# caidj0/Raytracer-2025

Hardware: NVIDIA B200
Metric: paths_per_sec (higher is better)
Workload: dtype f64

## Files before the change

### raytracer-2025_b200/csrc/api.cu

```cuda
#include <cuda_runtime.h>

#include <algorithm>
#include <cstdio>
#include <cstdlib>
#include <cstring>
#include <memory>
#include <mutex>
#include <new>
#include <string>
#include <thread>
#include <vector>

#include "compile.h"
#include "kernels.h"
#include "rt2025.h"

using namespace rt;

namespace {

thread_local std::string g_err;

int set_err(int code, const std::string& msg) {
    g_err = msg;
// ... 255 lines not shown
            if (!cs.nodes4.empty() && cs.nodes.size() * sizeof(Node) <= 2 * budget && stacks + cs.nodes4.size() * sizeof(Node4) > budget &&
                !getenv("RT2025_WIDE_BVH")) {
                RawVec<Node4>().swap(cs.nodes4);
                cs.world_root4 = INVALID_REF;
            }
        }
        s = new rt_scene();
        s->device = device;
        s->sm_count = sms;
        SceneView& v = s->view;
        keep_pool_memory(device);
        {
            cudaStream_t st = cudaStreamPerThread;
            Arena a;
            a.reserve(cs.nodes4), a.reserve(cs.nodes), a.reserve(cs.geom), a.reserve(cs.meta), a.reserve(cs.xforms), a.reserve(cs.materials), a.reserve(cs.textures);
            a.reserve(cs.images), a.reserve(cs.texels), a.reserve(cs.perlins), a.reserve(cs.media), a.reserve(cs.lights), a.reserve(cs.remaps);
            a.allocate(st);
            s->arena = a.base;
            v.nodes4 = a.put(cs.nodes4, st), v.world_root4 = cs.world_root4;
            v.nodes = a.put(cs.nodes, st), v.geom = a.put(cs.geom, st), v.meta = a.put(cs.meta, st), v.xforms = a.put(cs.xforms, st);
            v.materials = a.put(cs.materials, st), v.textures = a.put(cs.textures, st), v.images = a.put(cs.images, st);
            v.texels = a.put(cs.texels, st), v.perlins = a.put(cs.perlins, st), v.media = a.put(cs.media, st);
            v.lights = a.put(cs.lights, st), v.remaps = a.put(cs.remaps, st);
            CU(cudaStreamSynchronize(st));
        }
        v.world_root = cs.world_root;
        v.n_media = (uint32_t)cs.media.size();
        v.n_xforms = (uint32_t)cs.xforms.size();
        v.kinds = (cs.n_spheres && !cs.n_planars) ? 1u : ((cs.n_planars && !cs.n_spheres) ? 2u : 0u);
        v.n_lights = (uint32_t)cs.lights.size();
        v.n_prims = (uint32_t)cs.geom.size();
        s->ranks = cs.ranks;
        for (auto& m : cs.media) s->generic_media |= m.single_sphere == RT_NONE;
        v.media_xform = 0;
        for (auto& m : cs.media)
            if (m.xform != RT_NONE || (m.single_sphere != RT_NONE && cs.meta[m.single_sphere].xform != RT_NONE)) v.media_xform = 1;
        for (auto& m : cs.materials) s->class_mask |= 1u << m.shade_class;
        for (auto& t : cs.textures) s->black_texture.push_back(t.kind == RT_TEX_SOLID && t.color[0] == 0.0 && t.color[1] == 0.0 && t.color[2] == 0.0);
// ... 377 lines not shown
        CU(cudaEventRecord(ev[1], st));
        CU(cudaEventSynchronize(ev[1]));
        CU(cudaGetLastError());
        if (stats) {
            float ms = 0;
            CU(cudaEventElapsedTime(&ms, ev[0], ev[1]));
            const Counters zero{};
            const Counters& c = final_counters ? *final_counters : zero;
            stats->paths = nominal_paths;
            stats->segments = total_paths ? c.segments : 0;
            stats->node_visits = total_paths ? c.node_visits : 0;
            stats->prim_tests = total_paths ? c.prim_tests : 0;
            stats->errors = total_paths ? c.errors : 0;
            stats->iterations = total_paths ? c.iterations : 0;
            stats->reserved[0] = total_paths ? c.walk_segments : 0;
            stats->kernel_launches = launches;
            stats->ms_total = ms;
            stats->ms_raygen = ms_gen, stats->ms_extend = ms_ext, stats->ms_shade = ms_shd;
            stats->ms_other = ms_med;
        }
    } catch (const CudaFail& f) {
        rc = set_err(RT_ERR_CUDA, f.what);
    }
    for (auto& e : ev)
        if (e) cudaEventDestroy(e);
    return rc;
}

int rt_render(const rt_scene* s, const rt_camera* cam, const rt_render_opts* opts, void* accum, rt_stats* stats) {
    if (!s || !cam || !accum) return set_err(RT_ERR_INVALID, "null argument");
// ... 272 lines not shown
```

### raytracer-2025_b200/csrc/compile.cpp

```cpp
#include "compile.h"

#include <omp.h>

#include <memory>
#include <parallel/algorithm>

#include <chrono>
#include <cstdio>
#include <cstdlib>

#include <vector_functions.h>

#include <algorithm>
#include <cmath>
#include <cstring>
#include <limits>

namespace rt {

namespace {

struct V3 {
    double x, y, z;
};
// ... 968 lines not shown
            Medium& med = out.media[m];
            med.n_entry = MEDIUM_NO_ENTRIES;
            if (!(med.flags & MEDIUM_THICK) || getenv("RT2025_WALK_NO_ENTRIES")) continue;
            GroupBox b = group_boxes[group_of_medium[m]];
            for (int k = 0; k < 3; k++) {
                const float pad = 1e-4f * std::max(1.0f, std::max(std::fabs(b.lo[k]), std::fabs(b.hi[k])));
                b.lo[k] -= pad, b.hi[k] += pad;
            }
            uint32_t n = 0;
            const double* g = out.geom[med.single_sphere].d;
            const bool plain = med.xform == RT_NONE && out.meta[med.single_sphere].xform == RT_NONE && g[3] == 0.0 && g[4] == 0.0 && g[5] == 0.0;
            const double ball[4] = {g[0], g[1], g[2], std::fabs(g[6]) * (1.0 + 1e-4) + 1e-4};
            if (overlapping_leaves(b, plain ? ball : nullptr, out.world_root, med.entry, n)) med.n_entry = n;
            if (timer.on) fprintf(stderr, "[rt2025 compile] medium %zu is optically thick: %d entry leaves\n", m, (int)med.n_entry);
        }
        return RT_OK;
    }
};

}

int compile_scene(const rt_scene_desc& d, uint32_t flags, CompiledScene& out, std::string& err, WorldBuilder world_builder) {
    Compiler c{d, flags, out, err};
    c.world_builder = world_builder;
    return c.run();
}

}
```

### raytracer-2025_b200/csrc/compile.h

```cpp
#pragma once
#include <memory>
#include <string>
#include <type_traits>
#include <utility>
#include <vector>

#include <vector_types.h>

#include "rt2025.h"
#include "scene_types.h"

namespace rt {

template <class T, class A = std::allocator<T>>
struct default_init_allocator : A {
    using A::A;
    template <class U>
    struct rebind {
        using other = default_init_allocator<U, typename std::allocator_traits<A>::template rebind_alloc<U>>;
    };
    template <class U>
    void construct(U* p) noexcept(std::is_nothrow_default_constructible<U>::value) {
        ::new (static_cast<void*>(p)) U;
    }
// ... 10 lines not shown
    RawVec<Node4> nodes4;
    uint32_t world_root4 = INVALID_REF;
    uint32_t bvh4_depth = 0;
    RawVec<PrimGeom> geom;
    RawVec<PrimMeta> meta;
    std::vector<Xform> xforms;
    std::vector<Material> materials;
    std::vector<Texture> textures;
    std::vector<Image> images;
    std::vector<float4> texels;
    std::vector<Perlin> perlins;
    std::vector<Medium> media;
    std::vector<Light> lights;
    std::vector<Remap> remaps;
    std::vector<uint32_t> ranks;
    uint32_t world_root = INVALID_REF;
    uint32_t bvh_depth = 0;
    uint32_t media_bvh_depth = 0;
    uint32_t n_spheres = 0, n_planars = 0;
};

struct BuildBox;
using WorldBuilder = bool (*)(const RawVec<BuildBox>& boxes, uint32_t first_prim_base, RawVec<Node>& nodes,
                              RawVec<uint32_t>& order, uint32_t& depth_out, uint32_t& root_out);

int compile_scene(const rt_scene_desc& d, uint32_t flags, CompiledScene& out, std::string& err, WorldBuilder world_builder = nullptr);

uint32_t collapse_bvh4(const RawVec<Node>& nodes, uint32_t root, RawVec<Node4>& out, uint32_t& depth_out);

struct BuildBox {
// ... 9 lines not shown
```

### raytracer-2025_b200/csrc/kernels.cu

```cuda
#include <cuda_runtime.h>
#include <stdint.h>

#include <algorithm>

#include "kernels.h"
#include "shade.cuh"

namespace rt {

struct RayArrayIO {
    const SceneView& sv;
    const rt_ray* __restrict__ rays;
    rt_hit* __restrict__ out;
    double tmin, tmax;
    __device__ __forceinline__ double t_min() const { return tmin; }
    __device__ __forceinline__ bool load(uint32_t i, RayD& r, double& t1, uint32_t& prim0, uint32_t& rank0) const {
        const double* rp = reinterpret_cast<const double*>(rays + i);
        r.o = D3{rp[0], rp[1], rp[2]};
        r.d = D3{rp[3], rp[4], rp[5]};
        r.time = rp[6];
        t1 = tmax;
        prim0 = 0xFFFFFFFFu, rank0 = 0xFFFFFFFFu;
        return true;
    }
// ... 163 lines not shown
struct MediumDraws {
    Rand2 pair;
    uint32_t slot = 0xFFFFFFFFu;
    __device__ __forceinline__ double get(uint64_t seed, uint32_t pixel, uint32_t sample, uint32_t segment, uint32_t medium_index) {
        const uint32_t s = RT_MEDIUM_SLOT(medium_index);
        if (s != slot) {
            pair = philox_pair(seed, pixel, sample, segment, s);
            slot = s;
        }
        return (medium_index & 1u) ? pair.b : pair.a;
    }
};

constexpr uint32_t MEDIUM_INCUMBENT = 0x80000000u;

template <bool COUNT, bool XF>
__device__ __forceinline__ bool sample_sphere_medium(const SceneView& sv, const Medium& med, const RayD& r, double xi, double& tm, TraceCounters* cnt) {
    RayD lr = r;
    if (XF && med.xform != RT_NONE) lr = ray_to_local(sv, med.xform, r);
    RayD br = lr;
    if (XF) {
        const uint32_t bx = sv.meta[med.single_sphere].xform;
        if (bx != med.xform) br = bx == RT_NONE ? r : ray_to_local(sv, bx, r);
    }
    double t1, t2;
    if (COUNT) cnt->prims += 2;
    if (!sphere_entry_exit(sv.geom[med.single_sphere].d, br, t1, t2)) return false;
    if (t1 < 1e-8) t1 = 1e-8;
    if (t1 >= t2) return false;
    if (t1 < 0.0) t1 = 0.0;
    const double ray_length = length(lr.d);
    const double distance_inside_boundary = (t2 - t1) * ray_length;
    const float hf = (float)med.neg_inv_density * logf((float)xi);
    const float hf_err = 4e-7f * fabsf((float)med.neg_inv_density);
    if (hf > (float)distance_inside_boundary * 1.001f + hf_err) return false;
    const double hit_distance = med.neg_inv_density * log(xi);
    if (hit_distance > distance_inside_boundary) return false;
    tm = t1 + hit_distance / ray_length;
    return true;
}

template <bool COUNT, int MEDIA>
struct PathIO {
    const SceneView& sv;
    const RayRec* __restrict__ rays;
    HitRec* __restrict__ hits;
    uint8_t* __restrict__ cls;
    uint64_t seed;
    bool bin_by_class, drop_misses;
    TraceCounters* cnt;
    __device__ __forceinline__ double t_min() const { return 1e-8; }
    __device__ __forceinline__ bool load(uint32_t j, RayD& r, double& t1, uint32_t& prim0, uint32_t& rank0) const {
        uint64_t ids;
        load_ray(rays + j, r, ids);
// ... 70 lines not shown
template <bool COUNT, bool GENERIC, bool XF, int FILTER = 0>
__device__ __forceinline__ bool sample_media(const SceneView& sv, uint64_t seed, const RayD& r, uint32_t pixel, uint32_t sample, uint32_t segment, double& t,
                                             uint32_t& prim, uint32_t& kind, const float4* s_mem, uint32_t* stack, int stride, TraceCounters* cntp,
                                             uint32_t first, MediumDraws& draws) {
    uint32_t rank = kind == HIT_SURFACE ? sv.meta[prim].rank : (kind == HIT_MEDIUM ? sv.media[prim].rank : 0xFFFFFFFFu);
    bool changed = false;
        for (uint32_t k = 0; k < sv.n_media; k++) {
            uint32_t m = first + k;
            if (m >= sv.n_media) m -= sv.n_media;
            if (FILTER && ((sv.media[m].flags & MEDIUM_THICK) != 0u) != (FILTER == 1)) continue;
            const Medium& med = sv.media[m];
            const double xi = draws.get(seed, pixel, sample, segment, med.medium_index);
            double tm;
            RayD lr = r;
            if (XF && med.xform != RT_NONE) lr = ray_to_local(sv, med.xform, r);
            if (RT_MEDIA_EARLY_SCREEN && kind != HIT_MISS) {
                const float hf = (float)med.neg_inv_density * logf((float)xi);
                const float hf_err = 4e-7f * fabsf((float)med.neg_inv_density);
                const float len_f = sqrtf((float)lr.d.x * (float)lr.d.x + (float)lr.d.y * (float)lr.d.y + (float)lr.d.z * (float)lr.d.z);
                if (hf > (float)t * len_f * 1.001f + hf_err) continue;
            }
            if (med.single_sphere != RT_NONE) {
                if (!sample_sphere_medium<COUNT, XF>(sv, med, r, xi, tm, cntp)) continue;
            } else if (GENERIC) {
                double t1, t2;
                uint32_t bp;
                if (!closest_hit<COUNT, false>(sv, med.root, r, -INFINITY, INFINITY, s_mem, stack, stride, t1, bp, cntp)) continue;
                if (!closest_hit<COUNT, false>(sv, med.root, r, t1 + 0.0001, INFINITY, s_mem, stack, stride, t2, bp, cntp)) continue;
                if (t1 < 1e-8) t1 = 1e-8;
                if (t1 >= t2) continue;
                if (t1 < 0.0) t1 = 0.0;
                const double ray_length = length(lr.d);
                const double distance_inside_boundary = (t2 - t1) * ray_length;
                const double hit_distance = med.neg_inv_density * log(xi);
                if (hit_distance > distance_inside_boundary) continue;
                tm = t1 + hit_distance / ray_length;
// ... 437 lines not shown
        __syncthreads();
        if (q == 0) {
            store_ray(W.ray_q[W.parity ^ 1u] + npos, nr, pack_ids(pixel, sidx, segment + 1));
            store_beta(W.beta_q[W.parity ^ 1u] + npos, nbeta);
        }
    }
}

#ifndef RT_WALK_BLOCK
#define RT_WALK_BLOCK 128
#endif
constexpr int WALK_BLOCK = RT_WALK_BLOCK;
#ifndef RT_WALK_MIN_BLOCKS
#define RT_WALK_MIN_BLOCKS 4
#endif
template <bool XF, bool ENTRIES>
__global__ void __launch_bounds__(WALK_BLOCK, RT_WALK_MIN_BLOCKS) k_walk(SceneView sv, RenderParams P, WavefrontState W) {
    extern __shared__ float4 s_mem[];
    uint32_t* stack = reinterpret_cast<uint32_t*>(s_mem) + threadIdx.x;
    const uint32_t n = W.counters->n_shade[SC_WALK];
    const RayRec* __restrict__ rays = W.ray_q[W.parity];
    const BetaRec* __restrict__ betas = W.beta_q[W.parity];
    const uint32_t* __restrict__ queue = W.q_shade[SC_WALK];
    const uint32_t lane = threadIdx.x & 31u;
    const unsigned FULL = 0xFFFFFFFFu, lt_mask = (1u << lane) - 1u;
    TraceCounters cnt{0, 0};
    unsigned long long walked = 0;
    bool have = false;
    RayD r;
    D3 beta;
    uint32_t pixel = 0, sidx = 0, segment = 0, medium = 0;
    double t = 0.0;
    const uint32_t max_steps = n <= P.walk_drain_queue ? P.walk_drain_steps : 0xFFFFFFFFu;
    uint32_t steps = 0;
// ... 29 lines not shown
                const double2 b0 = sp2[0], b1 = sp2[1];
                beta = D3{b0.x, b0.y, b1.x};
                const double2 hw = *reinterpret_cast<const double2*>(W.hit_q + pos);
                t = hw.x;
                medium = (uint32_t)__double2hiint(hw.y);
                have = true;
                steps = 0;
            }
            pool_next += take;
            need = __ballot_sync(FULL, !have);
        }
        if (need == FULL) break;
        if (have) {
            RayD nr;
            D3 nbeta;
            if (!shade_one<SC_ISOTROPIC>(sv, P, W, r, beta, pixel, sidx, segment, t, medium, HIT_MEDIUM, nr, nbeta)) {
                have = false;
            } else {
                double tn = INFINITY;
                uint32_t pn = 0xFFFFFFFFu, kn = HIT_MISS;
                MediumDraws draws;
                sample_media<false, false, XF, 1>(sv, P.seed, nr, pixel, sidx, segment + 1u, tn, pn, kn, s_mem, stack, WALK_BLOCK, &cnt, medium, draws);
                bool stay = kn == HIT_MEDIUM && ++steps < max_steps;
                if (stay) {
                    sample_media<false, false, XF, 2>(sv, P.seed, nr, pixel, sidx, segment + 1u, tn, pn, kn, s_mem, stack, WALK_BLOCK, &cnt, 0u, draws);
                    stay = (sv.media[pn].flags & MEDIUM_THICK) != 0u;
                }
                if (stay) {
                    const Medium& mn = sv.media[pn];
                    const uint32_t med_rank = mn.rank;
                    double ts;
                    uint32_t ps;
                    if (ENTRIES || (pn == medium && mn.n_entry != MEDIUM_NO_ENTRIES)) {
                        for (uint32_t e = 0; e < mn.n_entry && stay; e++) stay = !leaf_beats_scatter(sv, mn.entry[e], nr, 1e-8, tn, med_rank);
                    } else if (closest_hit<false, true>(sv, sv.world_root, nr, 1e-8, tn, s_mem, stack, WALK_BLOCK, ts, ps, &cnt)) {
                        stay = !(ts < tn || sv.meta[ps].rank < med_rank);
                    }
                }
                if (stay) {
                    r = nr, beta = nbeta, segment++, t = tn, medium = pn;
                    walked++;
                } else {
                    const uint32_t npos = queue_reserve(&W.counters->n_extend[W.parity ^ 1u], 0);
                    store_ray(W.ray_q[W.parity ^ 1u] + npos, nr, pack_ids(pixel, sidx, segment + 1u));
                    store_beta(W.beta_q[W.parity ^ 1u] + npos, nbeta);
                    have = false;
                }
            }
        }
    }
    if (walked) {
        atomicAdd(&W.counters->segments, walked);
        atomicAdd(&W.counters->walk_segments, walked);
    }
}
static void launch_walk(const SceneView& sv, const RenderParams& P, const WavefrontState& W, int grid, cudaStream_t s) {
    SceneView wv = sv;
    wv.n_cached_nodes = 0;
    const size_t smem = (size_t)std::max(sv.tail_stack_entries, 4u) * WALK_BLOCK * sizeof(uint32_t);
    auto k = sv.media_xform ? (sv.walk_entries_only ? k_walk<true, true> : k_walk<true, false>) : (sv.walk_entries_only ? k_walk<false, true> : k_walk<false, false>);
    k<<<grid, WALK_BLOCK, smem, s>>>(wv, P, W);
}

constexpr int TAIL_BLOCK = MEDIA_BLOCK;
__global__ void __launch_bounds__(TAIL_BLOCK, 1) k_tail(SceneView sv, RenderParams P, WavefrontState W, uint32_t threshold) {
    extern __shared__ float4 s_mem[];
    uint32_t* stack = reinterpret_cast<uint32_t*>(s_mem) + threadIdx.x;
    Counters* c = W.counters;
    if (blockIdx.x == 0 && threadIdx.x == 0) reset_consumed_queues(W);
    const uint32_t np = W.parity ^ 1u;
    const uint32_t n = c->n_extend[np];
    if (n == 0 || n > threshold || c->next_path < W.total_paths) return;
    const RayRec* __restrict__ rays = W.ray_q[np];
// ... 233 lines not shown
```

### raytracer-2025_b200/csrc/kernels.h

```cpp
#pragma once
#include <cuda_runtime.h>
#include <stdint.h>

#include "rt2025.h"
#include "scene_types.h"

namespace rt {

#ifndef RT_EXTEND_BLOCK
#define RT_EXTEND_BLOCK 512
#endif
#ifndef RT_EXTEND_MIN_BLOCKS
#define RT_EXTEND_MIN_BLOCKS 1
#endif
constexpr int EXTEND_BLOCK = RT_EXTEND_BLOCK;
constexpr int EXTEND_MIN_BLOCKS = RT_EXTEND_MIN_BLOCKS;
constexpr size_t EXTEND_SMEM_MAX = 227 * 1024;
constexpr int SHADE_BLOCK = 256;
constexpr int MEDIA_BLOCK = 256;
#ifndef RT_REFILL_MIN
#define RT_REFILL_MIN 32
#endif
constexpr int REFILL_MIN = RT_REFILL_MIN;
#ifndef RT_SLAB_SIGNSEL
// ... 54 lines not shown
struct alignas(16) HitRec {
    double t;
    uint32_t kind, prim;
};
static_assert(sizeof(RayRec) == 64 && sizeof(BetaRec) == 32 && sizeof(HitRec) == 16, "stream record sizes");
constexpr uint32_t IDS_PIXEL_BITS = 28, IDS_SAMPLE_BITS = 24, IDS_SEGMENT_BITS = 12;

struct Counters {
    uint32_t n_extend[2];
    uint32_t n_shade[SC_COUNT];
    uint32_t n_pixels, pad;
    uint32_t n_unsampled, pad3;
    uint32_t gen_done, walk_cursor;
    unsigned long long next_path, segments, iterations, errors, node_visits, prim_tests;
    unsigned long long walk_segments;
};

struct WavefrontState {
    RayRec* ray_q[2];
    BetaRec* beta_q[2];
    HitRec* hit_q;
    uint8_t* cls_q;
    uint32_t* q_shade[SC_COUNT];
    uint32_t* pixel_list;
    double* accum;
    Counters* counters;
    uint32_t capacity, n_pixels;
    uint64_t total_paths;
    uint32_t parity, pad;
};
// ... 38 lines not shown
```

### raytracer-2025_b200/csrc/scene_types.h

```cpp
#pragma once
#include <stdint.h>

namespace rt {

constexpr uint32_t LEAF_FLAG = 0x80000000u;
constexpr uint32_t INVALID_REF = 0x7FFFFFFFu;
constexpr int MAX_LEAF_PRIMS = 8;
constexpr int TRAVERSAL_STACK = 64;
constexpr uint32_t META_MAT_MASK = 0x03FFFFFFu;
constexpr uint32_t META_CLASS_SHIFT = 26;

struct alignas(32) Node {
    float lo0[3], hi0[3];
    float lo1[3], hi1[3];
    uint32_t child0, child1;
    uint32_t pad0, pad1;
};
static_assert(sizeof(Node) == 64, "node must be 64 bytes");

struct alignas(32) Node4 {
    float box[4][6];
    uint32_t child[4];
    uint32_t pad[4];
};
// ... 67 lines not shown
    uint32_t single_sphere;
    uint32_t flags;
    uint32_t n_entry;
    uint32_t entry[MEDIUM_MAX_ENTRIES];
    uint32_t pad;
};
constexpr uint32_t MEDIUM_THICK = 1u;

struct Light {
    PrimGeom g;
    uint32_t kind;
    uint32_t xform;
    double weight, cdf, area;
};

enum ShadeClass : uint32_t {
    SC_MISS = 0,
    SC_DIFFUSE = 1,
    SC_TEXTURED = 2,
    SC_ISOTROPIC = 3,
    SC_METAL = 4,
    SC_DIELECTRIC = 5,
    SC_EMISSIVE = 6,
    SC_DISNEY = 7,
    SC_OTHER = 8,
    SC_WALK = 9,
    SC_COUNT = 10
};

struct SceneView {
// ... 14 lines not shown
    uint32_t media_xform;
    uint32_t world_root;
    uint32_t n_media, n_lights, n_prims;
    uint32_t n_nodes;
    uint32_t n_cached_nodes;
    uint32_t stack_entries;
    uint32_t l2_window_bytes;
    uint32_t park_leaves;
    uint32_t refill_min;
    uint32_t media_stack_entries;
    uint32_t tail_stack_entries;
    uint32_t kinds;
    uint32_t n_xforms;
    uint32_t walk_entries_only;
    uint32_t fifo_slots;
};

}
```

### raytracer-2025_b200/csrc/shade.cuh

```cuda
#pragma once
#include "disney.cuh"
#include "traverse.cuh"

namespace rt {

__device__ __forceinline__ int32_t as_i32_sat(double x) {
    if (isnan(x)) return 0;
    if (x >= 2147483647.0) return 2147483647;
    if (x <= -2147483648.0) return (-2147483647 - 1);
    return (int32_t)x;
}
__device__ __forceinline__ uint32_t as_u32_sat(double x) {
    if (!(x > 0.0)) return 0u;
    if (x >= 4294967295.0) return 0xFFFFFFFFu;
    return (uint32_t)x;
}

__device__ inline double perlin_noise(const Perlin* __restrict__ tab, D3 p) {
    double fx = floor(p.x), fy = floor(p.y), fz = floor(p.z);
    long long i = (long long)fx, j = (long long)fy, k = (long long)fz;
    double u = p.x - fx, v = p.y - fy, w = p.z - fz;
    double uu = u * u * (3.0 - 2.0 * u), vv = v * v * (3.0 - 2.0 * v), ww = w * w * (3.0 - 2.0 * w);
    double accum = 0.0;
#pragma unroll
// ... 145 lines not shown
    D3 n;
    ok = unit_vector((1.0 - h.u - h.v) * ld3(rm.normal[0]) + h.u * ld3(rm.normal[1]) + h.v * ld3(rm.normal[2]), n);
    if (rm.normal_tex != RT_NONE) {
        D3 c = texture_value(sv, rm.normal_tex, tex_coord.x, tex_coord.y, h.p);
        c = c * 2.0 - D3{1.0, 1.0, 1.0};
        if (!rm.has_uv_vecs) ok = false;
        D3 raw = ld3(rm.u_vec) * c.x + ld3(rm.v_vec) * c.y + n * c.z;
        ok = unit_vector(raw, n) && ok;
    }
    h.normal = n;
    h.u = tex_coord.x;
    h.v = tex_coord.y;
    return ok;
}

__device__ inline double light_leaf_pdf(const SceneView& sv, const Light& l, D3 origin, D3 direction) {
    if (l.xform != RT_NONE) {
        const Xform* x = sv.xforms + l.xform;
        for (uint32_t k = 0; k < x->n_chain; k++) {
            XformParams p = load_xform(sv.xforms + x->chain[k]);
            D3 lo = xf_detransform(p, origin);
            D3 lt = xf_detransform(p, origin + direction);
            origin = lo;
            direction = lt - lo;
        }
    }
    RayD r{origin, direction, 0.0};
    const double* g = l.g.d;
    if (l.kind == PRIM_SPHERE) {
        double t;
        if (!sphere_hit(g, r, 1e-8, INFINITY, t)) return 0.0;
        D3 center = ld3(g);
        double radius = g[6];
        double dist_squared = length_squared((center + 0.0 * ld3(g + 3)) - origin);
        double cos_theta_max = sqrt(1.0 - radius * radius / dist_squared);
        if (isnan(cos_theta_max)) return 1.0 / (4.0 * RT_PI);
        double solid_angle = 2.0 * RT_PI * (1.0 - cos_theta_max);
        return 1.0 / solid_angle;
    }
    Planar pl;
    load_planar(g, pl);
    double t, a, b2;
    if (!planar_hit_loaded(pl, l.kind == PRIM_TRIANGLE, r, 1e-8, INFINITY, t, a, b2)) return 0.0;
    double distance_squared = t * t * length_squared(direction);
    double cosine = fabs(dot(direction, pl.n) / length(direction));
    return distance_squared / (cosine * l.area);
}

__device__ inline double lights_pdf_value(const SceneView& sv, uint32_t lights_flat, D3 origin, D3 direction) {
    double sum = 0.0;
    if (lights_flat) {
        for (uint32_t i = 0; i < sv.n_lights; i++) sum += light_leaf_pdf(sv, sv.lights[i], origin, direction);
        return sum / (double)sv.n_lights;
    }
    for (uint32_t i = 0; i < sv.n_lights; i++) sum += sv.lights[i].weight * light_leaf_pdf(sv, sv.lights[i], origin, direction);
    return sum;
// ... 101 lines not shown
```

### raytracer-2025_b200/csrc/traverse.cuh

```cuda
#pragma once
#include "device_math.cuh"
#include "scene_types.h"

namespace rt {

struct RayD {
    D3 o, d;
    double time;
};

struct Quat {
    double w, x, y, z;
};
__device__ __forceinline__ Quat qmul(Quat a, Quat b) {
    return Quat{a.w * b.w - a.x * b.x - a.y * b.y - a.z * b.z, a.w * b.x + a.x * b.w + a.y * b.z - a.z * b.y,
                a.w * b.y - a.x * b.z + a.y * b.w + a.z * b.x, a.w * b.z + a.x * b.y - a.y * b.x + a.z * b.w};
}
__device__ __forceinline__ D3 qrotate(Quat q, D3 v) {
    Quat r = qmul(qmul(q, Quat{0.0, v.x, v.y, v.z}), Quat{q.w, -q.x, -q.y, -q.z});
    return D3{r.x, r.y, r.z};
}
struct XformParams {
    D3 offset, scale;
    Quat q;
// ... 99 lines not shown
    asm volatile("ld.global.nc.v8.f32 {%0,%1,%2,%3,%4,%5,%6,%7}, [%8];"
                 : "=f"(a.x), "=f"(a.y), "=f"(a.z), "=f"(a.w), "=f"(b.x), "=f"(b.y), "=f"(b.z), "=f"(b.w)
                 : "l"(p));
#else
    a = __ldg(reinterpret_cast<const float4*>(p)), b = __ldg(reinterpret_cast<const float4*>(p) + 1);
#endif
}
__device__ __forceinline__ void ldg256(const void* p, double2& a, double2& b) {
#if RT_LDG256
    asm volatile("ld.global.nc.v4.f64 {%0,%1,%2,%3}, [%4];" : "=d"(a.x), "=d"(a.y), "=d"(b.x), "=d"(b.y) : "l"(p));
#else
    a = __ldg(reinterpret_cast<const double2*>(p)), b = __ldg(reinterpret_cast<const double2*>(p) + 1);
#endif
}

__device__ __forceinline__ bool sphere_hit(const double* __restrict__ g, const RayD& r, double tmin, double tmax, double& t_out) {
    double2 a0, a1, a2, a3;
    ldg256(g, a0, a1);
    ldg256(g + 4, a2, a3);
    D3 center = D3{a0.x, a0.y, a1.x}, cvec = D3{a1.y, a2.x, a2.y};
    double radius = a3.x;
    D3 current_center = center + r.time * cvec;
    D3 oc = current_center - r.o;
    double a = length_squared(r.d);
    double h = dot(r.d, oc);
    double c = length_squared(oc) - radius * radius;
    double discriminant = h * h - a * c;
    if (discriminant < 0.0) return false;
    double sqrtd = sqrt(discriminant);
    double root = (h - sqrtd) / a;
    if (!contains(tmin, tmax, root)) {
        root = (h + sqrtd) / a;
        if (!contains(tmin, tmax, root)) return false;
    }
    t_out = root;
    return true;
}

struct Planar {
    D3 q, u, v, n, w;
    double D;
};
__device__ __forceinline__ void load_planar(const double* __restrict__ g, Planar& p) {
    const double2* s = reinterpret_cast<const double2*>(g);
    double2 a0 = __ldg(s), a1 = __ldg(s + 1), a2 = __ldg(s + 2), a3 = __ldg(s + 3);
    double2 a4 = __ldg(s + 4), a5 = __ldg(s + 5), a6 = __ldg(s + 6), a7 = __ldg(s + 7);
    p.q = D3{a0.x, a0.y, a1.x};
    p.u = D3{a1.y, a2.x, a2.y};
    p.v = D3{a3.x, a3.y, a4.x};
    p.n = D3{a4.y, a5.x, a5.y};
    p.D = a6.x;
    p.w = D3{a6.y, a7.x, a7.y};
}
__device__ __forceinline__ bool planar_hit_loaded(const Planar& p, bool triangle, const RayD& r, double tmin, double tmax,
                                                  double& t_out, double& alpha, double& beta) {
    double denom = dot(p.n, r.d);
    if (fabs(denom) < 1e-8) return false;
    double t = (p.D - dot(p.n, r.o)) / denom;
    if (!contains(tmin, tmax, t)) return false;
    D3 intersection = r.o + t * r.d;
    D3 hp = intersection - p.q;
    alpha = dot(p.w, cross(hp, p.v));
    beta = dot(p.w, cross(p.u, hp));
    if (!contains(0.0, 1.0, alpha) || !contains(0.0, 1.0, beta)) return false;
    if (triangle && !contains(0.0, 1.0, alpha + beta)) return false;
    t_out = t;
    return true;
// ... 491 lines not shown
                }
                parked = INVALID_REF;
                if (cur & LEAF_FLAG) {
                    parked = cur;
                    cur = sp > 0 ? stack[(--sp) * stride] : INVALID_REF;
                }
            }
            if (cur == INVALID_REF) {
                io.store(item, prim != 0xFFFFFFFFu, tbest, prim, prim_meta);
                have = false;
            }
        }
    }
}

__device__ __forceinline__ bool sphere_entry_exit(const double* __restrict__ g, const RayD& r, double& t1, double& t2) {
    const double2 a0 = __ldg(reinterpret_cast<const double2*>(g));
    const double2 a1 = __ldg(reinterpret_cast<const double2*>(g) + 1);
    const double2 a2 = __ldg(reinterpret_cast<const double2*>(g) + 2);
    const double2 a3 = __ldg(reinterpret_cast<const double2*>(g) + 3);
    D3 center = D3{a0.x, a0.y, a1.x}, cvec = D3{a1.y, a2.x, a2.y};
    double radius = a3.x;
    D3 current_center = center + r.time * cvec;
    D3 oc = current_center - r.o;
    double a = length_squared(r.d);
    double h = dot(r.d, oc);
    double c = length_squared(oc) - radius * radius;
    double discriminant = h * h - a * c;
    if (discriminant < 0.0) return false;
    double sqrtd = sqrt(discriminant);
    const double near_root = (h - sqrtd) / a, far_root = (h + sqrtd) / a;
    double first = near_root;
    if (!contains(-INFINITY, INFINITY, first)) {
        first = far_root;
        if (!contains(-INFINITY, INFINITY, first)) return false;
    }
    const double lo = first + 0.0001;
    double second = near_root;
    if (!contains(lo, INFINITY, second)) {
        second = far_root;
        if (!contains(lo, INFINITY, second)) return false;
    }
    t1 = first;
    t2 = second;
    return true;
}

}
```

### raytracer-2025_b200/rt2025.py

```python
import ctypes as C
import os
import subprocess

import numpy as np

PKG_DIR = os.path.dirname(os.path.abspath(__file__))
ROOT = os.path.dirname(PKG_DIR)
RT_NONE = 0xFFFFFFFF
RT_OPT_COUNT = 1
RT_OPT_STAGE_TIMES = 2
RT_ACCUM_F32 = 0
RT_ACCUM_F64 = 1
RT_BUILD_NO_REF_RANKS = 1
RT_BUILD_DEVICE_LBVH = 2

ABI_SYMBOLS = [
    "rt_scene_create", "rt_scene_destroy", "rt_closest_hit", "rt_closest_hit_device", "rt_render",
    "rt_render_device", "rt_render_rgb8", "rt_render_multi", "rt_render_multi_rgb8", "rt_tonemap", "rt_tonemap_device", "rt_scene_get_info", "rt_scene_get_ranks", "rt_last_error",
    "rt_abi_version", "rt_device_count",
]


class RtError(RuntimeError):
    pass
# ... 27 lines not shown
class rt_stats(C.Structure):
    _fields_ = [
        ("paths", C.c_uint64), ("segments", C.c_uint64), ("node_visits", C.c_uint64),
        ("prim_tests", C.c_uint64), ("errors", C.c_uint64), ("kernel_launches", C.c_uint64),
        ("ms_total", C.c_double), ("ms_raygen", C.c_double), ("ms_extend", C.c_double),
        ("ms_shade", C.c_double), ("ms_other", C.c_double), ("iterations", C.c_uint64),
        ("reserved", C.c_uint64 * 4),
    ]

    def as_dict(self):
        return {k: getattr(self, k) for k, _ in self._fields_ if k != "reserved"}

    @property
    def walk_segments(self):
        return int(self.reserved[0])


class rt_scene_info(C.Structure):
    _fields_ = [
        ("n_prims", C.c_uint32), ("n_spheres", C.c_uint32), ("n_planars", C.c_uint32), ("n_nodes", C.c_uint32),
        ("n_media", C.c_uint32), ("n_lights", C.c_uint32), ("n_materials", C.c_uint32), ("n_textures", C.c_uint32),
        ("bvh_depth", C.c_uint32), ("node_bytes", C.c_uint32), ("device_bytes", C.c_uint64),
    ]


class rth_camera_params(C.Structure):
    _fields_ = [
        ("aspect_ratio", C.c_double), ("image_width", C.c_uint32), ("samples_per_pixel", C.c_uint32),
        ("max_depth", C.c_uint32), ("background_tex", C.c_uint32), ("vertical_fov_in_degrees", C.c_double),
        ("look_from", C.c_double * 3), ("look_at", C.c_double * 3), ("vec_up", C.c_double * 3),
# ... 396 lines not shown
```

Before: 1.366 billion.

## Add lean random-walk kernel with scene data staged in shared memory

Adds a specialized random-walk path for optically thick media. It applies when the scene has few media, lights and entry primitives, all untransformed. At compile time the relevant light, sphere and primitive data are packed into a compact WalkLean struct, which each walk block copies into shared memory. The walk then does isotropic scattering, light sampling, media competition and exit tests directly against this small set, instead of going through generic shading and BVH-based media sampling. This removes global loads and traversal per walk step, but it adds a per-block copy into shared memory, a separate kernel variant and a larger grid.

```diff
diff --git a/raytracer-2025_b200/csrc/api.cu b/raytracer-2025_b200/csrc/api.cu
--- a/raytracer-2025_b200/csrc/api.cu
+++ b/raytracer-2025_b200/csrc/api.cu
@@ -293,14 +293,14 @@
             cudaStream_t st = cudaStreamPerThread;
             Arena a;
             a.reserve(cs.nodes4), a.reserve(cs.nodes), a.reserve(cs.geom), a.reserve(cs.meta), a.reserve(cs.xforms), a.reserve(cs.materials), a.reserve(cs.textures);
-            a.reserve(cs.images), a.reserve(cs.texels), a.reserve(cs.perlins), a.reserve(cs.media), a.reserve(cs.lights), a.reserve(cs.remaps);
+            a.reserve(cs.images), a.reserve(cs.texels), a.reserve(cs.perlins), a.reserve(cs.media), a.reserve(cs.lights), a.reserve(cs.remaps), a.reserve(cs.walk_lean);
             a.allocate(st);
             s->arena = a.base;
             v.nodes4 = a.put(cs.nodes4, st), v.world_root4 = cs.world_root4;
             v.nodes = a.put(cs.nodes, st), v.geom = a.put(cs.geom, st), v.meta = a.put(cs.meta, st), v.xforms = a.put(cs.xforms, st);
             v.materials = a.put(cs.materials, st), v.textures = a.put(cs.textures, st), v.images = a.put(cs.images, st);
             v.texels = a.put(cs.texels, st), v.perlins = a.put(cs.perlins, st), v.media = a.put(cs.media, st);
-            v.lights = a.put(cs.lights, st), v.remaps = a.put(cs.remaps, st);
+            v.lights = a.put(cs.lights, st), v.remaps = a.put(cs.remaps, st), v.walk_lean = a.put(cs.walk_lean, st);
             CU(cudaStreamSynchronize(st));
         }
         v.world_root = cs.world_root;
@@ -708,6 +708,7 @@
             stats->errors = total_paths ? c.errors : 0;
             stats->iterations = total_paths ? c.iterations : 0;
             stats->reserved[0] = total_paths ? c.walk_segments : 0;
+            stats->reserved[1] = total_paths ? c.walk_lean_segments : 0;
             stats->kernel_launches = launches;
             stats->ms_total = ms;
             stats->ms_raygen = ms_gen, stats->ms_extend = ms_ext, stats->ms_shade = ms_shd;
diff --git a/raytracer-2025_b200/csrc/compile.cpp b/raytracer-2025_b200/csrc/compile.cpp
--- a/raytracer-2025_b200/csrc/compile.cpp
+++ b/raytracer-2025_b200/csrc/compile.cpp
@@ -1006,7 +1006,51 @@
             if (overlapping_leaves(b, plain ? ball : nullptr, out.world_root, med.entry, n)) med.n_entry = n;
             if (timer.on) fprintf(stderr, "[rt2025 compile] medium %zu is optically thick: %d entry leaves\n", m, (int)med.n_entry);
         }
+        walk_lean();
+        if (timer.on) fprintf(stderr, "[rt2025 compile] random walk: %s\n", out.walk_lean.empty() ? "generic" : (out.walk_lean[0].shell != RT_NONE ? "lean, shell" : "lean"));
         return RT_OK;
+    }
+
+    void walk_lean() {
+        out.walk_lean.clear();
+        const size_t n_media = out.media.size(), n_lights = out.lights.size();
+        if (n_media > WALK_LEAN_MEDIA || n_lights > WALK_LEAN_LIGHTS) return;
+        WalkLean L;
+        std::memset(&L, 0, sizeof(L));
+        L.n_media = (uint32_t)n_media, L.n_lights = (uint32_t)n_lights, L.thick = RT_NONE, L.shell = RT_NONE;
+        for (size_t m = 0; m < n_media; m++) {
+            const Medium& med = out.media[m];
+            if (med.single_sphere == RT_NONE || med.xform != RT_NONE || out.meta[med.single_sphere].xform != RT_NONE) return;
+            if (med.flags & MEDIUM_THICK) {
+                if (L.thick != RT_NONE || med.n_entry == MEDIUM_NO_ENTRIES) return;
+                L.thick = (uint32_t)m;
+            }
+            std::memcpy(L.sphere[m], out.geom[med.single_sphere].d, 7 * sizeof(double));
+            L.neg_inv_density[m] = med.neg_inv_density;
+            L.rank[m] = med.rank, L.medium_index[m] = med.medium_index;
+        }
+        if (L.thick == RT_NONE) return;
+        const Medium& thick = out.media[L.thick];
+        const Material& iso = out.materials[thick.material];
+        if (iso.kind != RT_MAT_ISOTROPIC || iso.tex >= out.textures.size() || out.textures[iso.tex].kind != RT_TEX_SOLID) return;
+        for (int k = 0; k < 3; k++) L.axp[k] = (1.0 / (4.0 * 3.14159265358979323846264338327950288)) * out.textures[iso.tex].color[k];
+        for (size_t i = 0; i < n_lights; i++) {
+            const Light& l = out.lights[i];
+            if (l.xform != RT_NONE || l.weight != 1.0 / (double)n_lights) return;
+            L.lights[i] = l;
+        }
+        for (uint32_t e = 0; e < thick.n_entry; e++) {
+            const uint32_t first = (thick.entry[e] & ~LEAF_FLAG) >> 3, count = (thick.entry[e] & 7u) + 1;
+            for (uint32_t pi = first; pi < first + count; pi++) {
+                const PrimMeta& pm = out.meta[pi];
+                if (L.n_prims == WALK_LEAN_PRIMS || pm.xform != RT_NONE) return;
+                const uint32_t k = L.n_prims++;
+                L.prim[k] = out.geom[pi];
+                L.prim_kind[k] = pm.kind_mat >> 30, L.prim_rank[k] = pm.rank;
+                if (L.shell == RT_NONE && L.prim_kind[k] == PRIM_SPHERE && std::memcmp(out.geom[pi].d, L.sphere[L.thick], 7 * sizeof(double)) == 0) L.shell = k;
+            }
+        }
+        out.walk_lean.push_back(L);
     }
 };
 
diff --git a/raytracer-2025_b200/csrc/compile.h b/raytracer-2025_b200/csrc/compile.h
--- a/raytracer-2025_b200/csrc/compile.h
+++ b/raytracer-2025_b200/csrc/compile.h
@@ -48,6 +48,7 @@
     std::vector<Light> lights;
     std::vector<Remap> remaps;
     std::vector<uint32_t> ranks;
+    std::vector<WalkLean> walk_lean;
     uint32_t world_root = INVALID_REF;
     uint32_t bvh_depth = 0;
     uint32_t media_bvh_depth = 0;
diff --git a/raytracer-2025_b200/csrc/kernels.cu b/raytracer-2025_b200/csrc/kernels.cu
--- a/raytracer-2025_b200/csrc/kernels.cu
+++ b/raytracer-2025_b200/csrc/kernels.cu
@@ -201,6 +201,28 @@
 
 constexpr uint32_t MEDIUM_INCUMBENT = 0x80000000u;
 
+__device__ __forceinline__ bool medium_free_flight(double t1, double t2, const RayD& lr, double neg_inv_density, double xi, double& tm) {
+    if (t1 < 1e-8) t1 = 1e-8;
+    if (t1 >= t2) return false;
+    if (t1 < 0.0) t1 = 0.0;
+    const double ray_length = length(lr.d);
+    const double distance_inside_boundary = (t2 - t1) * ray_length;
+    const float hf = (float)neg_inv_density * logf((float)xi);
+    const float hf_err = 4e-7f * fabsf((float)neg_inv_density);
+    if (hf > (float)distance_inside_boundary * 1.001f + hf_err) return false;
+    const double hit_distance = neg_inv_density * log(xi);
+    if (hit_distance > distance_inside_boundary) return false;
+    tm = t1 + hit_distance / ray_length;
+    return true;
+}
+
+__device__ __forceinline__ bool free_flight_overshoots(double neg_inv_density, double xi, double t, const D3& ld) {
+    const float hf = (float)neg_inv_density * logf((float)xi);
+    const float hf_err = 4e-7f * fabsf((float)neg_inv_density);
+    const float len_f = sqrtf((float)ld.x * (float)ld.x + (float)ld.y * (float)ld.y + (float)ld.z * (float)ld.z);
+    return hf > (float)t * len_f * 1.001f + hf_err;
+}
+
 template <bool COUNT, bool XF>
 __device__ __forceinline__ bool sample_sphere_medium(const SceneView& sv, const Medium& med, const RayD& r, double xi, double& tm, TraceCounters* cnt) {
     RayD lr = r;
@@ -213,18 +235,7 @@
     double t1, t2;
     if (COUNT) cnt->prims += 2;
     if (!sphere_entry_exit(sv.geom[med.single_sphere].d, br, t1, t2)) return false;
-    if (t1 < 1e-8) t1 = 1e-8;
-    if (t1 >= t2) return false;
-    if (t1 < 0.0) t1 = 0.0;
-    const double ray_length = length(lr.d);
-    const double distance_inside_boundary = (t2 - t1) * ray_length;
-    const float hf = (float)med.neg_inv_density * logf((float)xi);
-    const float hf_err = 4e-7f * fabsf((float)med.neg_inv_density);
-    if (hf > (float)distance_inside_boundary * 1.001f + hf_err) return false;
-    const double hit_distance = med.neg_inv_density * log(xi);
-    if (hit_distance > distance_inside_boundary) return false;
-    tm = t1 + hit_distance / ray_length;
-    return true;
+    return medium_free_flight(t1, t2, lr, med.neg_inv_density, xi, tm);
 }
 
 template <bool COUNT, int MEDIA>
@@ -325,12 +336,7 @@
             double tm;
             RayD lr = r;
             if (XF && med.xform != RT_NONE) lr = ray_to_local(sv, med.xform, r);
-            if (RT_MEDIA_EARLY_SCREEN && kind != HIT_MISS) {
-                const float hf = (float)med.neg_inv_density * logf((float)xi);
-                const float hf_err = 4e-7f * fabsf((float)med.neg_inv_density);
-                const float len_f = sqrtf((float)lr.d.x * (float)lr.d.x + (float)lr.d.y * (float)lr.d.y + (float)lr.d.z * (float)lr.d.z);
-                if (hf > (float)t * len_f * 1.001f + hf_err) continue;
-            }
+            if (RT_MEDIA_EARLY_SCREEN && kind != HIT_MISS && free_flight_overshoots(med.neg_inv_density, xi, t, lr.d)) continue;
             if (med.single_sphere != RT_NONE) {
                 if (!sample_sphere_medium<COUNT, XF>(sv, med, r, xi, tm, cntp)) continue;
             } else if (GENERIC) {
@@ -798,10 +804,109 @@
 #ifndef RT_WALK_MIN_BLOCKS
 #define RT_WALK_MIN_BLOCKS 4
 #endif
-template <bool XF, bool ENTRIES>
-__global__ void __launch_bounds__(WALK_BLOCK, RT_WALK_MIN_BLOCKS) k_walk(SceneView sv, RenderParams P, WavefrontState W) {
+#ifndef RT_WALK_LEAN_MIN_BLOCKS
+#define RT_WALK_LEAN_MIN_BLOCKS 4
+#endif
+
+__device__ __forceinline__ bool walk_lean_segment(const SceneView& sv, const WalkLean& L, const RenderParams& P, const WavefrontState& W, const RayD& r,
+                                                  D3 beta, uint32_t pixel, uint32_t sidx, uint32_t segment, double t, uint32_t max_steps,
+                                                  uint32_t& steps, RayD& nr, D3& nbeta, double& tn, bool& stay) {
+    stay = false;
+    nr.o = r.o + t * r.d;
+    nr.time = r.time;
+    const Rand2 pick = philox_pair(P.seed, pixel, sidx, segment, RT_SLOT_MIXTURE);
+    const Rand2 dx = philox_pair(P.seed, pixel, sidx, segment, RT_SLOT_DIRECTION);
+    const uint32_t n_lights = L.n_lights;
+    D3 gen = D3{0.0, 0.0, 0.0};
+    bool panic = false;
+    if (n_lights > 0 && !(pick.a < 0.5)) {
+        uint32_t leaf = n_lights - 1;
+        for (uint32_t i = 0; i < n_lights; i++)
+            if (pick.b < L.lights[i].cdf) {
+                leaf = i;
+                break;
+            }
+        panic = !light_leaf_random(L.lights[leaf], nr.o, dx.a, dx.b, gen);
+    } else {
+        gen = random_unit_vector(dx.a, dx.b);
+    }
+    const double value0 = 1.0 / (4.0 * RT_PI);
+    double pdf_val = value0;
+    if (!panic && n_lights > 0) {
+        double sum = 0.0;
+        for (uint32_t i = 0; i < n_lights; i++) sum += light_leaf_pdf<true>(sv, L.lights[i], nr.o, gen);
+        const double value1 = n_lights == 1 ? sum : sum / (double)n_lights;
+        if (isnan(value1) || (value0 == 0.0 && value1 == 0.0))
+            panic = true;
+        else
+            pdf_val = value0 * 0.5 + value1 * 0.5;
+    }
+    if (panic || pdf_val == 0.0) {
+        atomicAdd(&W.counters->errors, 1ull);
+        return false;
+    }
+    nr.d = gen;
+    nbeta = beta * (ld3(L.axp) / pdf_val);
+    if (segment + 1 >= P.cam.max_depth || (nbeta.x == 0.0 && nbeta.y == 0.0 && nbeta.z == 0.0)) return false;
+
+    const uint32_t seg1 = segment + 1u, thick = L.thick;
+    MediumDraws draws;
+    double near_root, far_root;
+    {
+        const double* s = L.sphere[thick];
+        double t1, t2;
+        const double xi = draws.get(P.seed, pixel, sidx, seg1, L.medium_index[thick]);
+        const bool inside = sphere_entry_exit_at(ld3(s), ld3(s + 3), s[6], nr, t1, t2, near_root, far_root);
+        if (!inside || !medium_free_flight(t1, t2, nr, L.neg_inv_density[thick], xi, tn)) return true;
+    }
+    if (!(++steps < max_steps)) return true;
+    const uint32_t med_rank = L.rank[thick];
+    for (uint32_t m = 0; m < L.n_media; m++) {
+        if (m == thick) continue;
+        const double xi = draws.get(P.seed, pixel, sidx, seg1, L.medium_index[m]);
+        if (RT_MEDIA_EARLY_SCREEN && free_flight_overshoots(L.neg_inv_density[m], xi, tn, nr.d)) continue;
+        const double* s = L.sphere[m];
+        double t1, t2, nroot, froot, tm;
+        if (!sphere_entry_exit_at(ld3(s), ld3(s + 3), s[6], nr, t1, t2, nroot, froot) || !medium_free_flight(t1, t2, nr, L.neg_inv_density[m], xi, tm)) continue;
+        if (tm < tn || (tm == tn && L.rank[m] < med_rank)) return true;
+    }
+    bool beaten = false;
+    for (uint32_t i = 0; i < L.n_prims && !beaten; i++) {
+        const double* g = L.prim[i].d;
+        double th;
+        bool hit;
+        if (i == L.shell) {
+            th = near_root;
+            hit = contains(1e-8, tn, th);
+            if (!hit) {
+                th = far_root;
+                hit = contains(1e-8, tn, th);
+            }
+        } else if (L.prim_kind[i] == PRIM_SPHERE) {
+            hit = sphere_hit_at(ld3(g), ld3(g + 3), g[6], nr, 1e-8, tn, th);
+        } else {
+            Planar pl;
+            load_planar_plain(g, pl);
+            double a, b;
+            hit = planar_hit_loaded(pl, L.prim_kind[i] == PRIM_TRIANGLE, nr, 1e-8, tn, th, a, b);
+        }
+        beaten = hit && (th < tn || L.prim_rank[i] < med_rank);
+    }
+    stay = !beaten;
+    return true;
+}
+
+template <bool XF, bool ENTRIES, bool LEAN = false>
+__global__ void __launch_bounds__(WALK_BLOCK, LEAN ? RT_WALK_LEAN_MIN_BLOCKS : RT_WALK_MIN_BLOCKS) k_walk(SceneView sv, RenderParams P, WavefrontState W) {
     extern __shared__ float4 s_mem[];
     uint32_t* stack = reinterpret_cast<uint32_t*>(s_mem) + threadIdx.x;
+    const WalkLean& L = *reinterpret_cast<const WalkLean*>(s_mem);
+    if (LEAN) {
+        unsigned long long* dst = reinterpret_cast<unsigned long long*>(s_mem);
+        const unsigned long long* src = reinterpret_cast<const unsigned long long*>(sv.walk_lean);
+        for (uint32_t k = threadIdx.x; k < sizeof(WalkLean) / 8; k += WALK_BLOCK) dst[k] = src[k];
+        __syncthreads();
+    }
     const uint32_t n = W.counters->n_shade[SC_WALK];
     const RayRec* __restrict__ rays = W.ray_q[W.parity];
     const BetaRec* __restrict__ betas = W.beta_q[W.parity];
@@ -861,14 +966,17 @@
         if (have) {
             RayD nr;
             D3 nbeta;
-            if (!shade_one<SC_ISOTROPIC>(sv, P, W, r, beta, pixel, sidx, segment, t, medium, HIT_MEDIUM, nr, nbeta)) {
-                have = false;
-            } else {
-                double tn = INFINITY;
-                uint32_t pn = 0xFFFFFFFFu, kn = HIT_MISS;
+            double tn = INFINITY;
+            uint32_t pn = medium;
+            bool alive, stay = false;
+            if constexpr (LEAN) {
+                alive = walk_lean_segment(sv, L, P, W, r, beta, pixel, sidx, segment, t, max_steps, steps, nr, nbeta, tn, stay);
+            } else if ((alive = shade_one<SC_ISOTROPIC>(sv, P, W, r, beta, pixel, sidx, segment, t, medium, HIT_MEDIUM, nr, nbeta))) {
+                uint32_t kn = HIT_MISS;
+                pn = 0xFFFFFFFFu;
                 MediumDraws draws;
                 sample_media<false, false, XF, 1>(sv, P.seed, nr, pixel, sidx, segment + 1u, tn, pn, kn, s_mem, stack, WALK_BLOCK, &cnt, medium, draws);
-                bool stay = kn == HIT_MEDIUM && ++steps < max_steps;
+                stay = kn == HIT_MEDIUM && ++steps < max_steps;
                 if (stay) {
                     sample_media<false, false, XF, 2>(sv, P.seed, nr, pixel, sidx, segment + 1u, tn, pn, kn, s_mem, stack, WALK_BLOCK, &cnt, 0u, draws);
                     stay = (sv.media[pn].flags & MEDIUM_THICK) != 0u;
@@ -884,26 +992,33 @@
                         stay = !(ts < tn || sv.meta[ps].rank < med_rank);
                     }
                 }
-                if (stay) {
-                    r = nr, beta = nbeta, segment++, t = tn, medium = pn;
-                    walked++;
-                } else {
-                    const uint32_t npos = queue_reserve(&W.counters->n_extend[W.parity ^ 1u], 0);
-                    store_ray(W.ray_q[W.parity ^ 1u] + npos, nr, pack_ids(pixel, sidx, segment + 1u));
-                    store_beta(W.beta_q[W.parity ^ 1u] + npos, nbeta);
-                    have = false;
-                }
+            }
+            if (!alive) {
+                have = false;
+            } else if (stay) {
+                r = nr, beta = nbeta, segment++, t = tn, medium = pn;
+                walked++;
+            } else {
+                const uint32_t npos = queue_reserve(&W.counters->n_extend[W.parity ^ 1u], 0);
+                store_ray(W.ray_q[W.parity ^ 1u] + npos, nr, pack_ids(pixel, sidx, segment + 1u));
+                store_beta(W.beta_q[W.parity ^ 1u] + npos, nbeta);
+                have = false;
             }
         }
     }
     if (walked) {
         atomicAdd(&W.counters->segments, walked);
         atomicAdd(&W.counters->walk_segments, walked);
+        if (LEAN) atomicAdd(&W.counters->walk_lean_segments, walked);
     }
 }
 static void launch_walk(const SceneView& sv, const RenderParams& P, const WavefrontState& W, int grid, cudaStream_t s) {
     SceneView wv = sv;
     wv.n_cached_nodes = 0;
+    if (sv.walk_lean) {
+        k_walk<false, true, true><<<grid / RT_WALK_MIN_BLOCKS * RT_WALK_LEAN_MIN_BLOCKS, WALK_BLOCK, sizeof(WalkLean), s>>>(wv, P, W);
+        return;
+    }
     const size_t smem = (size_t)std::max(sv.tail_stack_entries, 4u) * WALK_BLOCK * sizeof(uint32_t);
     auto k = sv.media_xform ? (sv.walk_entries_only ? k_walk<true, true> : k_walk<true, false>) : (sv.walk_entries_only ? k_walk<false, true> : k_walk<false, false>);
     k<<<grid, WALK_BLOCK, smem, s>>>(wv, P, W);
diff --git a/raytracer-2025_b200/csrc/kernels.h b/raytracer-2025_b200/csrc/kernels.h
--- a/raytracer-2025_b200/csrc/kernels.h
+++ b/raytracer-2025_b200/csrc/kernels.h
@@ -92,6 +92,7 @@
     uint32_t gen_done, walk_cursor;
     unsigned long long next_path, segments, iterations, errors, node_visits, prim_tests;
     unsigned long long walk_segments;
+    unsigned long long walk_lean_segments;
 };
 
 struct WavefrontState {
diff --git a/raytracer-2025_b200/csrc/scene_types.h b/raytracer-2025_b200/csrc/scene_types.h
--- a/raytracer-2025_b200/csrc/scene_types.h
+++ b/raytracer-2025_b200/csrc/scene_types.h
@@ -105,6 +105,21 @@
     double weight, cdf, area;
 };
 
+constexpr uint32_t WALK_LEAN_MEDIA = 4, WALK_LEAN_LIGHTS = 4, WALK_LEAN_PRIMS = 8;
+struct WalkLean {
+    Light lights[WALK_LEAN_LIGHTS];
+    PrimGeom prim[WALK_LEAN_PRIMS];
+    double sphere[WALK_LEAN_MEDIA][8];
+    double neg_inv_density[WALK_LEAN_MEDIA];
+    double axp[3];
+    double pad0;
+    uint32_t rank[WALK_LEAN_MEDIA], medium_index[WALK_LEAN_MEDIA];
+    uint32_t prim_kind[WALK_LEAN_PRIMS], prim_rank[WALK_LEAN_PRIMS];
+    uint32_t n_media, thick, n_lights, n_prims;
+    uint32_t shell;
+    uint32_t pad1[3];
+};
+
 enum ShadeClass : uint32_t {
     SC_MISS = 0,
     SC_DIFFUSE = 1,
@@ -149,6 +164,7 @@
     uint32_t n_xforms;
     uint32_t walk_entries_only;
     uint32_t fifo_slots;
+    const WalkLean* walk_lean;
 };
 
 }
diff --git a/raytracer-2025_b200/csrc/shade.cuh b/raytracer-2025_b200/csrc/shade.cuh
--- a/raytracer-2025_b200/csrc/shade.cuh
+++ b/raytracer-2025_b200/csrc/shade.cuh
@@ -183,8 +183,9 @@
     return ok;
 }
 
+template <bool STAGED = false>
 __device__ inline double light_leaf_pdf(const SceneView& sv, const Light& l, D3 origin, D3 direction) {
-    if (l.xform != RT_NONE) {
+    if (!STAGED && l.xform != RT_NONE) {
         const Xform* x = sv.xforms + l.xform;
         for (uint32_t k = 0; k < x->n_chain; k++) {
             XformParams p = load_xform(sv.xforms + x->chain[k]);
@@ -198,7 +199,7 @@
     const double* g = l.g.d;
     if (l.kind == PRIM_SPHERE) {
         double t;
-        if (!sphere_hit(g, r, 1e-8, INFINITY, t)) return 0.0;
+        if (!(STAGED ? sphere_hit_at(ld3(g), ld3(g + 3), g[6], r, 1e-8, INFINITY, t) : sphere_hit(g, r, 1e-8, INFINITY, t))) return 0.0;
         D3 center = ld3(g);
         double radius = g[6];
         double dist_squared = length_squared((center + 0.0 * ld3(g + 3)) - origin);
@@ -208,7 +209,10 @@
         return 1.0 / solid_angle;
     }
     Planar pl;
-    load_planar(g, pl);
+    if (STAGED)
+        load_planar_plain(g, pl);
+    else
+        load_planar(g, pl);
     double t, a, b2;
     if (!planar_hit_loaded(pl, l.kind == PRIM_TRIANGLE, r, 1e-8, INFINITY, t, a, b2)) return 0.0;
     double distance_squared = t * t * length_squared(direction);
diff --git a/raytracer-2025_b200/csrc/traverse.cuh b/raytracer-2025_b200/csrc/traverse.cuh
--- a/raytracer-2025_b200/csrc/traverse.cuh
+++ b/raytracer-2025_b200/csrc/traverse.cuh
@@ -137,12 +137,7 @@
 #endif
 }
 
-__device__ __forceinline__ bool sphere_hit(const double* __restrict__ g, const RayD& r, double tmin, double tmax, double& t_out) {
-    double2 a0, a1, a2, a3;
-    ldg256(g, a0, a1);
-    ldg256(g + 4, a2, a3);
-    D3 center = D3{a0.x, a0.y, a1.x}, cvec = D3{a1.y, a2.x, a2.y};
-    double radius = a3.x;
+__device__ __forceinline__ bool sphere_hit_at(D3 center, D3 cvec, double radius, const RayD& r, double tmin, double tmax, double& t_out) {
     D3 current_center = center + r.time * cvec;
     D3 oc = current_center - r.o;
     double a = length_squared(r.d);
@@ -158,6 +153,12 @@
     }
     t_out = root;
     return true;
+}
+__device__ __forceinline__ bool sphere_hit(const double* __restrict__ g, const RayD& r, double tmin, double tmax, double& t_out) {
+    double2 a0, a1, a2, a3;
+    ldg256(g, a0, a1);
+    ldg256(g + 4, a2, a3);
+    return sphere_hit_at(D3{a0.x, a0.y, a1.x}, D3{a1.y, a2.x, a2.y}, a3.x, r, tmin, tmax, t_out);
 }
 
 struct Planar {
@@ -174,6 +175,11 @@
     p.n = D3{a4.y, a5.x, a5.y};
     p.D = a6.x;
     p.w = D3{a6.y, a7.x, a7.y};
+}
+__device__ __forceinline__ void load_planar_plain(const double* g, Planar& p) {
+    p.q = ld3(g), p.u = ld3(g + 3), p.v = ld3(g + 6), p.n = ld3(g + 9);
+    p.D = g[12];
+    p.w = ld3(g + 13);
 }
 __device__ __forceinline__ bool planar_hit_loaded(const Planar& p, bool triangle, const RayD& r, double tmin, double tmax,
                                                   double& t_out, double& alpha, double& beta) {
@@ -695,22 +701,18 @@
     }
 }
 
-__device__ __forceinline__ bool sphere_entry_exit(const double* __restrict__ g, const RayD& r, double& t1, double& t2) {
-    const double2 a0 = __ldg(reinterpret_cast<const double2*>(g));
-    const double2 a1 = __ldg(reinterpret_cast<const double2*>(g) + 1);
-    const double2 a2 = __ldg(reinterpret_cast<const double2*>(g) + 2);
-    const double2 a3 = __ldg(reinterpret_cast<const double2*>(g) + 3);
-    D3 center = D3{a0.x, a0.y, a1.x}, cvec = D3{a1.y, a2.x, a2.y};
-    double radius = a3.x;
+__device__ __forceinline__ bool sphere_entry_exit_at(D3 center, D3 cvec, double radius, const RayD& r, double& t1, double& t2, double& near_root,
+                                                     double& far_root) {
     D3 current_center = center + r.time * cvec;
     D3 oc = current_center - r.o;
     double a = length_squared(r.d);
     double h = dot(r.d, oc);
     double c = length_squared(oc) - radius * radius;
     double discriminant = h * h - a * c;
+    near_root = far_root = __longlong_as_double(0x7FF8000000000000ll);
     if (discriminant < 0.0) return false;
     double sqrtd = sqrt(discriminant);
-    const double near_root = (h - sqrtd) / a, far_root = (h + sqrtd) / a;
+    near_root = (h - sqrtd) / a, far_root = (h + sqrtd) / a;
     double first = near_root;
     if (!contains(-INFINITY, INFINITY, first)) {
         first = far_root;
@@ -726,5 +728,13 @@
     t2 = second;
     return true;
 }
-
-}
+__device__ __forceinline__ bool sphere_entry_exit(const double* __restrict__ g, const RayD& r, double& t1, double& t2) {
+    const double2 a0 = __ldg(reinterpret_cast<const double2*>(g));
+    const double2 a1 = __ldg(reinterpret_cast<const double2*>(g) + 1);
+    const double2 a2 = __ldg(reinterpret_cast<const double2*>(g) + 2);
+    const double2 a3 = __ldg(reinterpret_cast<const double2*>(g) + 3);
+    double near_root, far_root;
+    return sphere_entry_exit_at(D3{a0.x, a0.y, a1.x}, D3{a1.y, a2.x, a2.y}, a3.x, r, t1, t2, near_root, far_root);
+}
+
+}
diff --git a/raytracer-2025_b200/rt2025.py b/raytracer-2025_b200/rt2025.py
--- a/raytracer-2025_b200/rt2025.py
+++ b/raytracer-2025_b200/rt2025.py
@@ -65,6 +65,10 @@
     @property
     def walk_segments(self):
         return int(self.reserved[0])
+
+    @property
+    def walk_lean_segments(self):
+        return int(self.reserved[1])
 
 
 class rt_scene_info(C.Structure):
```

Measured after the change: 1.507 billion (median of 6 runs). 10.3% higher.
